# HumanCompatibleAI/overcooked_ai

Measured on NVIDIA H100. Metric: env-steps/sec (joint transitions), higher is better.
Workload: dtype int32

## Files before the change

include/ovc_b200.h:

```cpp
#ifndef OVC_B200_H
#define OVC_B200_H

#include <stddef.h>
#include <stdint.h>

#ifdef __cplusplus
extern "C" {
#endif

#define OVC_ABI_VERSION 5

#define OVC_A_NORTH 0
#define OVC_A_SOUTH 1
#define OVC_A_EAST 2
#define OVC_A_WEST 3
#define OVC_A_STAY 4
#define OVC_A_INTERACT 5
#define OVC_NUM_ACTIONS 6

#define OVC_T_FLOOR 0
#define OVC_T_COUNTER 1
#define OVC_T_ONION 2
#define OVC_T_TOMATO 3
#define OVC_T_DISH 4
// ... 229 lines not shown
} ovc_episode_stats_t;
int ovc_record_transition_stats(const int32_t *sparse, const int32_t *shaped, const int32_t *done, const float *factor, int64_t n_envs,
                                float *rewards, uint8_t *dones, int64_t *ret_sparse, float *ret_mixed, const ovc_episode_stats_t *stats,
                                void *stream);

int ovc_policy_tail(const void *x, int64_t n_rows, int k0, float in_slope, const void *w_first, const float *b_first,
                    const void *w_hidden, const float *b_hidden, int n_hidden, const void *w_heads, const float *b_heads,
                    float slope, int n_actions, uint64_t seed, uint64_t *counter, int32_t *actions, float *values,
                    float *scores, void *stream);
int ovc_policy_tail_logp(const void *x, int64_t n_rows, int k0, float in_slope, const void *w_first, const float *b_first,
                         const void *w_hidden, const float *b_hidden, int n_hidden, const void *w_heads, const float *b_heads,
                         float slope, int n_actions, uint64_t seed, uint64_t *counter, int32_t *actions, float *values,
                         float *scores, float *logp, void *stream);
int ovc_policy_hidden(const void *x, int64_t n_rows, int k0, float in_slope, const void *w_first, const float *b_first,
                      const void *w_hidden, const float *b_hidden, int n_hidden, float slope, void *hidden, void *stream);
int ovc_policy_tail_view(const void *x, int64_t n_rows, int k0, float in_slope, const void *w_first, const float *b_first,
                         const void *w_hidden, const float *b_hidden, int n_hidden, const void *w_heads, const float *b_heads,
                         float slope, int n_actions, uint64_t seed, uint64_t *counter, const int32_t *swap, int seat, int32_t *actions,
                         float *values, float *scores, float *logp, void *stream);

int ovc_lstm_head(const void *x, const void *h_in, const float *c_in, const int32_t *reset, int64_t n_rows, const void *w,
                  const float *b, const void *w_heads, const float *b_heads, int n_actions, uint64_t seed, uint64_t *counter,
                  void *h_out, float *c_out, void *snap_h, float *snap_c, int32_t *actions, float *values, float *logp,
                  float *scores, void *stream);
int ovc_lstm_head_view(const void *x, const void *h_in, const float *c_in, const int32_t *reset, int64_t n_rows, const void *w,
                       const float *b, const void *w_heads, const float *b_heads, int n_actions, uint64_t seed, uint64_t *counter,
                       const int32_t *swap, int seat, void *h_out, float *c_out, void *snap_h, float *snap_c, int32_t *actions,
                       float *values, float *logp, float *scores, void *stream);
int ovc_record_transition_view(const int32_t *sparse, const int32_t *shaped, const int32_t *done, const float *factor, int64_t n_envs,
                               const int32_t *swap, int seat, float *rewards, uint8_t *dones, int64_t *ret_sparse, float *ret_mixed,
                               const ovc_episode_stats_t *stats, void *stream);
int ovc_gae_view(const float *rewards, const float *values, const uint8_t *dones, const float *last_values, int64_t n_steps,
                 int64_t n_envs, float gamma, float lambda, float *advantages, float *value_targets, void *stream);

int ovc_wide_layers(const void *a0, int64_t m, int k0, const void *w1, const float *b1, int n1, const void *w2, const float *b2,
                    int n2, float slope, void *z2, void *stream);

int ovc_partner_policy(const void *layouts, int n_layouts, const void *lut, const int32_t *state, const int32_t *partner_seat,
                       int64_t n_envs, int state_words, int n_features, int width, const void *w_first, const float *b_first,
                       const void *w_hidden, const float *b_hidden, int n_hidden, const void *w_heads, const float *b_heads, int n_actions,
                       uint64_t seed, uint64_t *counter, int32_t *actions, float *scores, void *stream);
int ovc_assign_partners(const int32_t *done, const float *bc_factor, int64_t n_envs, uint64_t seed, uint64_t *counter, int32_t *partner_seat,
                        void *stream);

int ovc_featurize(const void *layouts, int n_layouts, const void *lut, const int32_t *state,
                  const int32_t *view_swap, float *out, int64_t n_envs, int state_words, int num_pots,
                  void *stream);

int ovc_potential(const void *layouts, int n_layouts, const void *pot_tables, const void *cost_lut,
                  const double *gpow, int n_pow, const int32_t *state, double *out, int64_t n_envs,
                  int state_words, void *stream);
size_t ovc_potential_table_size(void);

#ifdef __cplusplus
}
#endif
#endif
```

overcooked_ai_b200/_native.py:

```python
import ctypes
import os

_HERE = os.path.dirname(os.path.abspath(__file__))
LIB_PATH = os.environ.get("OVC_B200_LIB") or os.path.join(_HERE, "csrc", "libovc_b200.so")

ABI_VERSION = 5
F_AUTO_RESET = 1
F_PDL = 2
F_ACT_U8 = 4
F_OUT_NARROW = 8
F_OUT_PACKED = 16
F_OUT_CODES = 32
F_ACT_PACKED = 64
F_OUT_STREAM = 128
F_STREAM_CAP_SHIFT = 16
STREAM_CAP_MAX = 0xFFFF
F_IO_SHIFT = 8
IO_DEFAULT, IO_TMA_TENSOR, IO_TMA_BULK, IO_DIRECT = 0, 1, 2, 3
DT_F32, DT_U8, DT_I32, DT_BF16 = 0, 1, 2, 3



class RandomStart(ctypes.Structure):
    _fields_ = [("seed", ctypes.c_uint64), ("obj_threshold", ctypes.c_uint32), ("random_start_pos", ctypes.c_int32),
# ... 24 lines not shown
    pass


def lib():
    global _lib
    if _lib is not None:
        return _lib
    if not os.path.exists(LIB_PATH):
        raise NativeLibraryError(
            "%s not found: the CUDA extension is not built (python -m overcooked_ai_b200.build). "
            "This engine has no CPU fallback." % LIB_PATH
        )
    L = ctypes.CDLL(LIB_PATH)
    vp, i32, i64 = ctypes.c_void_p, ctypes.c_int, ctypes.c_int64
    L.ovc_abi_version.restype = i32
    L.ovc_layout_table_size.restype = ctypes.c_size_t
    L.ovc_feat_lut_entry_size.restype = ctypes.c_size_t
    L.ovc_last_error.restype = ctypes.c_char_p
    L.ovc_step.argtypes = [vp, i32, vp, vp, vp, vp, vp, vp, vp, i64, i32, i32, i32, vp, vp]
    L.ovc_rollout.argtypes = [vp, i32, vp, vp, vp, vp, vp, vp, vp, i64, i32, i32, i32, i32, vp, vp]
    L.ovc_reset.argtypes = [vp, i32, vp, vp, vp, vp, i64, i32, vp, vp]
    L.ovc_encode_lossless.argtypes = [vp, i32, vp, vp, vp, i32, i64, i32, i32, i32, i32, vp]
    L.ovc_encode_linear.argtypes = [vp, i32, vp, vp, vp, vp, vp, i64, i32, i32, i32, i32, i32, ctypes.c_float, vp]
    L.ovc_sample_actions.argtypes = [vp, i32, i32, i64, ctypes.c_uint64, vp, vp, vp]
    L.ovc_accumulate_returns.argtypes = [vp, vp, ctypes.c_float, i64, vp, vp, vp]
    L.ovc_policy_tail.argtypes = [vp, i64, i32, ctypes.c_float, vp, vp, vp, vp, i32, vp, vp, ctypes.c_float, i32, ctypes.c_uint64, vp, vp, vp, vp, vp]
    L.ovc_policy_tail_logp.argtypes = L.ovc_policy_tail.argtypes[:-1] + [vp, vp]
    L.ovc_policy_hidden.argtypes = [vp, i64, i32, ctypes.c_float, vp, vp, vp, vp, i32, ctypes.c_float, vp, vp]
    L.ovc_lstm_head.argtypes = [vp, vp, vp, vp, i64, vp, vp, vp, vp, i32, ctypes.c_uint64, vp, vp, vp, vp, vp, vp, vp, vp, vp, vp]
    L.ovc_sample_actions_logp.argtypes = [vp, i32, i32, i64, ctypes.c_uint64, vp, vp, vp, vp]
    L.ovc_encode_linear_view.argtypes = [vp, i32, vp, vp, i32, vp, vp, vp, i64, i32, i32, i32, i32, i32, ctypes.c_float, vp]
    L.ovc_sample_actions_view.argtypes = [vp, i32, i32, i64, ctypes.c_uint64, vp, vp, i32, vp, vp, vp]
    L.ovc_policy_tail_view.argtypes = L.ovc_policy_tail.argtypes[:15] + [vp, i32, vp, vp, vp, vp, vp]
    L.ovc_lstm_head_view.argtypes = L.ovc_lstm_head.argtypes[:12] + [vp, i32] + L.ovc_lstm_head.argtypes[12:]
    L.ovc_record_transition.argtypes = [vp, vp, vp, vp, i64, vp, vp, vp, vp, vp]
    L.ovc_record_transition_stats.argtypes = [vp, vp, vp, vp, i64, vp, vp, vp, vp, ctypes.POINTER(EpisodeStatsDesc), vp]
    L.ovc_gae.argtypes = [vp, vp, vp, vp, i64, i64, ctypes.c_float, ctypes.c_float, vp, vp, vp]
    L.ovc_record_transition_view.argtypes = [vp, vp, vp, vp, i64, vp, i32, vp, vp, vp, vp, ctypes.POINTER(EpisodeStatsDesc), vp]
    L.ovc_gae_view.argtypes = L.ovc_gae.argtypes
    L.ovc_wide_layers.argtypes = [vp, i64, i32, vp, vp, i32, vp, vp, i32, ctypes.c_float, vp, vp]
    L.ovc_featurize.argtypes = [vp, i32, vp, vp, vp, vp, i64, i32, i32, vp]
    L.ovc_partner_policy.argtypes = [vp, i32, vp, vp, vp, i64, i32, i32, i32, vp, vp, vp, vp, i32, vp, vp, i32, ctypes.c_uint64, vp, vp, vp, vp]
    L.ovc_assign_partners.argtypes = [vp, vp, i64, ctypes.c_uint64, vp, vp, vp]
    L.ovc_potential.argtypes = [vp, i32, vp, vp, vp, i32, vp, vp, i64, i32, vp]
    L.ovc_potential_table_size.restype = ctypes.c_size_t
    L.ovc_expand_codes_host.argtypes = [vp, i64, i64, vp, vp, i32, vp, vp, vp, vp, i32]
    L.ovc_expand_stream_host.argtypes = [vp, vp, i64, i64, i64, i64, vp, vp, i32, vp, vp, vp, vp, i32, ctypes.POINTER(i64)]
    L.ovc_pipeline_create.argtypes = [ctypes.POINTER(PipelineDesc), ctypes.POINTER(vp)]
    L.ovc_pipeline_run.argtypes = [vp, vp, vp, vp, vp, vp, i32, vp, i32, ctypes.POINTER(i64)]
    L.ovc_pipeline_wait.argtypes = [vp, i64]
    L.ovc_pipeline_join.argtypes = [vp, vp]
    L.ovc_pipeline_destroy.argtypes = [vp]
    L.ovc_pipeline_destroy.restype = None
    for f in (L.ovc_step, L.ovc_rollout, L.ovc_reset, L.ovc_encode_lossless, L.ovc_encode_linear, L.ovc_sample_actions, L.ovc_accumulate_returns, L.ovc_policy_tail, L.ovc_wide_layers, L.ovc_featurize, L.ovc_potential,
              L.ovc_policy_tail_logp, L.ovc_policy_hidden, L.ovc_lstm_head,
              L.ovc_encode_linear_view, L.ovc_sample_actions_view, L.ovc_policy_tail_view, L.ovc_lstm_head_view, L.ovc_sample_actions_logp, L.ovc_record_transition, L.ovc_record_transition_stats, L.ovc_gae, L.ovc_record_transition_view, L.ovc_gae_view, L.ovc_partner_policy, L.ovc_assign_partners, L.ovc_expand_codes_host, L.ovc_expand_stream_host, L.ovc_pipeline_create, L.ovc_pipeline_run, L.ovc_pipeline_wait, L.ovc_pipeline_join):
        f.restype = i32
    if L.ovc_abi_version() != ABI_VERSION:
        raise NativeLibraryError("ABI version mismatch: library %d, binding %d" % (L.ovc_abi_version(), ABI_VERSION))
    _lib = L
    return L


EXPORTED_SYMBOLS = (
    "ovc_abi_version", "ovc_layout_table_size", "ovc_feat_lut_entry_size", "ovc_last_error",
    "ovc_step", "ovc_rollout", "ovc_reset", "ovc_encode_lossless", "ovc_encode_linear", "ovc_sample_actions", "ovc_accumulate_returns", "ovc_policy_tail", "ovc_wide_layers", "ovc_featurize", "ovc_potential",
    "ovc_potential_table_size", "ovc_expand_codes_host", "ovc_expand_stream_host",
    "ovc_policy_tail_logp", "ovc_sample_actions_logp", "ovc_record_transition", "ovc_record_transition_stats", "ovc_gae",
    "ovc_partner_policy", "ovc_assign_partners", "ovc_policy_hidden", "ovc_lstm_head",
    "ovc_encode_linear_view", "ovc_sample_actions_view", "ovc_policy_tail_view", "ovc_lstm_head_view",
    "ovc_record_transition_view", "ovc_gae_view",
    "ovc_pipeline_create", "ovc_pipeline_run", "ovc_pipeline_wait", "ovc_pipeline_join", "ovc_pipeline_destroy",
)


def check(rc):
    if rc != 0:
        raise RuntimeError("ovc native call failed (%d): %s" % (rc, lib().ovc_last_error().decode()))
```

overcooked_ai_b200/batched.py:

```python
import ctypes

import numpy as np
import torch

from overcooked_ai_b200 import _native
from overcooked_ai_b200 import layout as L

_TORCH_DT = {torch.float32: _native.DT_F32, torch.uint8: _native.DT_U8, torch.int32: _native.DT_I32,
             torch.bfloat16: _native.DT_BF16}


def _as_layouts(layouts, mdp_params):
    if isinstance(layouts, (str, L.CompiledLayout)) or hasattr(layouts, "compiled"):
        layouts = [layouts]
    out = []
    for l in layouts:
        if isinstance(l, str):
            l = L.compile_layout(l, **(mdp_params or {}))
        elif hasattr(l, "compiled"):
            l = l.compiled
        out.append(l)
    return out


class BatchedOvercookedEnv(object):
    def __init__(self, layouts, n_envs, horizon=400, device="cuda", auto_reset=False, state_words=None,
                 io=_native.IO_DEFAULT, env_layout=None, mdp_params=None, pdl=True,
                 random_start_pos=False, rnd_obj_prob_thresh=0.0, seed=0, random_layout=False):
        self._lib = _native.lib()
        if not torch.cuda.is_available():
            raise RuntimeError("BatchedOvercookedEnv needs a CUDA device: this engine has no CPU fallback")
        self.device = torch.device(device)
        if self.device.type != "cuda":
            raise ValueError("device must be a CUDA device")
        if self.device.index is None:
            self.device = torch.device("cuda", torch.cuda.current_device())
        self.layouts = _as_layouts(layouts, mdp_params)
        self.n_layouts = len(self.layouts)
        self._longest_cook = max(int(l.cook_time.max()) for l in self.layouts)
        self.n_envs = int(n_envs)
        self.horizon = int(horizon) if horizon < 2**31 else 0
        self.auto_reset = bool(auto_reset)
        self.io = int(io)
        self.pdl = bool(pdl)
        tab, starts, S = L.build_tables(self.layouts, state_words)
        assert tab.shape[1] == self._lib.ovc_layout_table_size(), "layout table size mismatch with the native library"
        self.state_words = S
        self._tab_host, self._starts_host = tab, starts
        with torch.cuda.device(self.device):
            self.tables = torch.from_numpy(tab).to(self.device)
            self.start_records = torch.from_numpy(starts).to(self.device)
            if env_layout is None:
# ... 65 lines not shown
        return (self.n_envs + 31) // 32

    def alloc_stream_out(self, T, cap, n_chunks=1, pin=False, dense_backup=False):
        G = self.n_groups()
        mk = (lambda sh, dt: torch.zeros(sh, dtype=dt, pin_memory=True)) if pin else (lambda sh, dt: torch.zeros(sh, dtype=dt, device=self.device))
        return (mk((T, G), torch.int32), mk((n_chunks, G, cap), torch.int16), mk((T, self.n_envs), torch.int16) if dense_backup else None)

    def rollout_stream(self, actions, cap, out=None, dense_backup=False):
        act_flag = self._action_flag(actions)
        T = actions.shape[0]
        assert 1 <= cap <= _native.STREAM_CAP_MAX
        if out is None:
            out = self.alloc_stream_out(T, cap, dense_backup=dense_backup)
        masks, values, dense = out
        assert masks.dtype == torch.int32 and tuple(masks.shape) == (T, self.n_groups()) and masks.is_cuda and masks.is_contiguous()
        assert values.dtype == torch.int16 and values.numel() == self.n_groups() * cap and values.is_cuda and values.is_contiguous()
        flags = self._flags() | act_flag | _native.F_OUT_STREAM | (int(cap) << _native.F_STREAM_CAP_SHIFT)
        if flags >= 2**31:
            flags -= 2**32
        _native.check(self._lib.ovc_rollout(
            self.tables.data_ptr(), self.n_layouts, self.start_records.data_ptr(), self.state.data_ptr(),
            actions.data_ptr(), values.data_ptr(), 0, 0 if dense is None else dense.data_ptr(), masks.data_ptr(),
            self.n_envs, T, self.state_words, self.horizon, flags, self._rs_ptr(), self._stream()))
        return out

    def expand_stream(self, masks, values, chunk=None, sparse=True, shaped=True, done=True, events=False, n_threads=0, out=None):
        assert masks.dtype == torch.int32 and not masks.is_cuda and masks.is_contiguous() and masks.dim() == 2
        assert values.dtype == torch.int16 and not values.is_cuda and values.is_contiguous() and values.dim() == 3
        T, G = masks.shape
        assert G == self.n_groups() and values.shape[1] == G
        chunk = T if chunk is None else int(chunk)
        assert values.shape[0] == -(-T // chunk)
        out, tbl, lay, ptrs = self._dense_host_out(T, out, sparse, shaped, done, events)
        over = ctypes.c_int64(0)
        _native.check(self._lib.ovc_expand_stream_host(
            masks.data_ptr(), values.data_ptr(), T, chunk, values.shape[2], self.n_envs, lay, tbl.ctypes.data, self.n_layouts, *ptrs,
            int(n_threads), ctypes.byref(over)))
        return out, int(over.value)

    def _dense_host_out(self, T, out, sparse, shaped, done, events):
        tbl = np.ascontiguousarray(self.code_reward_table(), dtype=np.int32)
        lay = self.env_layout_host.ctypes.data
        if self.random_layout:
            assert (tbl == tbl[:1]).all(), "random_layout with different reward tables: the codes alone do not name the layout"
            lay = 0
        if out is None:
            N = self.n_envs
            want = (("sparse", sparse, (T, N), torch.int16), ("shaped", shaped, (T, N, 2), torch.int8),
                    ("done", done, (T, N), torch.uint8), ("events", events, (T, N, 2), torch.int32))
            out = {k: torch.empty(shape, dtype=dt) for k, on, shape, dt in want if on}
        ptrs = [out[k].data_ptr() if k in out else 0 for k in ("sparse", "shaped", "done", "events")]
        return out, tbl, lay, ptrs

    def alloc_rollout_out(self, T, narrow=False, pin=False, packed=False, codes=False):
        N = self.n_envs
        mk = (lambda sh, dt: torch.empty(sh, dtype=dt, pin_memory=True)) if pin else (lambda sh, dt: torch.empty(sh, dtype=dt, device=self.device))
        if codes:
            return (None, None, None, mk((T, N), torch.int16))
        if packed:
            return (mk((T, N), torch.int16), mk((T, N, 2), torch.int8), None, mk((T, N), torch.int16))
        dts = (torch.int16, torch.int8, torch.uint8, torch.int32) if narrow else (torch.int32,) * 4
        shapes = ((T, N), (T, N, 2), (T, N), (T, N, 2))
        return tuple(mk(sh, dt) for sh, dt in zip(shapes, dts))

    def _action_flag(self, actions):
        assert actions.dtype in (torch.int32, torch.uint8) and actions.is_cuda and actions.is_contiguous() and actions.dim() in (2, 3)
        assert actions.shape[1] == self.n_envs
        if actions.dim() == 2:
            assert actions.dtype == torch.uint8, "one-byte joint actions are uint8 [T, N]"
            return _native.F_ACT_PACKED
        assert actions.shape[2] == 2
        return _native.F_ACT_U8 if actions.dtype == torch.uint8 else 0

    def rollout(self, actions, out=None):
        flags = self._flags() | self._action_flag(actions)
        T = actions.shape[0]
        if out is None:
            out = self.alloc_rollout_out(T)
        sparse, shaped, done, events = out
        if sparse is None:
            assert shaped is None and done is None and events.dtype == torch.int16 and events.dim() == 2
            assert tuple(events.shape) == (T, self.n_envs) and events.is_cuda and events.is_contiguous()
            flags |= _native.F_OUT_CODES
            _native.check(self._lib.ovc_rollout(
                self.tables.data_ptr(), self.n_layouts, self.start_records.data_ptr(), self.state.data_ptr(),
                actions.data_ptr(), 0, 0, 0, events.data_ptr(), self.n_envs, T, self.state_words, self.horizon, flags,
                self._rs_ptr(), self._stream()))
            return out
        if done is None:
            assert sparse.dtype == torch.int16 and shaped.dtype == torch.int8 and events.dtype == torch.int16 and events.dim() == 2
            assert self.narrow_ok(), "rewards of these layouts do not fit the narrow formats"
            flags |= _native.F_OUT_PACKED
        elif sparse.dtype == torch.int16:
            assert shaped.dtype == torch.int8 and done.dtype == torch.uint8 and events.dtype == torch.int32
            assert self.narrow_ok(), "rewards of these layouts do not fit the narrow formats"
            flags |= _native.F_OUT_NARROW
        else:
            assert sparse.dtype == shaped.dtype == done.dtype == events.dtype == torch.int32
        _native.check(self._lib.ovc_rollout(
            self.tables.data_ptr(), self.n_layouts, self.start_records.data_ptr(), self.state.data_ptr(),
            actions.data_ptr(), sparse.data_ptr(), shaped.data_ptr(), 0 if done is None else done.data_ptr(), events.data_ptr(),
            self.n_envs, T, self.state_words, self.horizon, flags, self._rs_ptr(), self._stream()))
        return out

    def code_reward_table(self):
        from overcooked_ai_b200 import wire

        return wire.code_reward_table(self.layouts)

    def expand_codes(self, evcode, sparse=True, shaped=True, done=True, events=False, n_threads=0, out=None):
        assert evcode.dtype == torch.int16 and not evcode.is_cuda and evcode.is_contiguous() and evcode.dim() == 2
        T, N = evcode.shape
        assert N == self.n_envs
        out, tbl, lay, ptrs = self._dense_host_out(T, out, sparse, shaped, done, events)
        _native.check(self._lib.ovc_expand_codes_host(evcode.data_ptr(), T, N, lay, tbl.ctypes.data, self.n_layouts, *ptrs, int(n_threads)))
        return out
# ... 261 lines not shown
        rec = (events >> L.EV_RECIPE_SHIFT) & 15
        ids = self.env_layout if layout_ids is None else layout_ids
        lid = ids.long().view(*([1] * (events.dim() - 2)), -1, 1).expand_as(rec)
        return val[lid, rec.long()] * ((events >> 15) & 1)

    def get_states(self, indices=None):
        recs = self.state.cpu().numpy()
        idx = range(self.n_envs) if indices is None else indices
        return [L.unpack_state(self.layouts[int(recs[i][3]) & 0xFF], recs[i]) for i in idx]

    def set_states(self, states, indices=None):
        idx = list(range(self.n_envs)) if indices is None else list(indices)
        lids = self._layout_ids_host()
        recs = np.stack([L.pack_state(self.layouts[lids[i]], s, int(lids[i]), self.state_words) for i, s in zip(idx, states)])
        self.state[torch.as_tensor(idx, device=self.device)] = torch.from_numpy(recs).to(self.device)


class PassTicket(object):

    def __init__(self, pipe, ticket):
        self._pipe, self.ticket = pipe, ticket

    def synchronize(self):
        _native.check(self._pipe._lib.ovc_pipeline_wait(self._pipe._handle, self.ticket))


class HostRolloutPipeline(object):

    def __init__(self, env, n_steps, chunk=50, narrow=False, packed=False, codes=False, host_buffers=1, stream=False,
                 stream_fill=0.25, packed_actions=True):
        codes = codes or stream
        narrow = narrow or packed or codes
        self.env, self.T, self.chunk, self.narrow, self.packed = env, int(n_steps), int(chunk), bool(narrow), bool(packed)
        self.codes, self.stream = bool(codes), bool(stream)
        self.packed_actions = bool(packed_actions) and self.codes
        if narrow:
            assert env.narrow_ok(), "rewards of these layouts do not fit the narrow formats"
        N, dev = env.n_envs, env.device
        self._lib = env._lib
        self.act_dtype = torch.uint8 if narrow else torch.int32
        self.act_shape = (N,) if self.packed_actions else (N, 2)
        self.n_chunks = -(-self.T // self.chunk)
        self.stream_cap = max(1, min(_native.STREAM_CAP_MAX, int(round(self.chunk * 32 * float(stream_fill))))) if stream else 0
        with torch.cuda.device(dev):
            self.d_act = [torch.empty((self.chunk,) + self.act_shape, dtype=self.act_dtype, device=dev) for _ in range(2)]
            if stream:
                G = env.n_groups()
                self.d_out = [(torch.empty((G, self.stream_cap), dtype=torch.int16, device=dev), None, None,
                               torch.empty((self.chunk, G), dtype=torch.int32, device=dev)) for _ in range(2)]
                self.d_codes_full = [torch.empty((self.T, N), dtype=torch.int16, device=dev) for _ in range(2)]
                self.h_outs = [(torch.zeros((self.n_chunks, G, self.stream_cap), dtype=torch.int16, pin_memory=True), None, None,
                                torch.zeros((self.T, G), dtype=torch.int32, pin_memory=True)) for _ in range(max(1, int(host_buffers)))]
            else:
                self.d_out = [env.alloc_rollout_out(self.chunk, narrow=narrow, packed=packed, codes=codes) for _ in range(2)]
                self.h_outs = [env.alloc_rollout_out(self.T, narrow=narrow, pin=True, packed=packed, codes=codes)
                               for _ in range(max(1, int(host_buffers)))]
        self.h_out = self.h_outs[0]
        self._runs = 0
        self.h2d_bytes_per_step = N * (1 if self.packed_actions else 2) * self.d_act[0].element_size()
        if stream:
            self.d2h_bytes_per_step = (self.h_out[3].numel() * 4 + self.h_out[0].numel() * 2) / float(self.T)
        else:
            self.d2h_bytes_per_step = sum(N * (2 if o.dim() == 3 else 1) * o.element_size() for o in self.h_out if o is not None)
        flags = env._flags() | (_native.F_ACT_PACKED if self.packed_actions else _native.F_ACT_U8 if narrow else 0)
        flags |= (_native.F_OUT_STREAM if stream else _native.F_OUT_CODES if codes else _native.F_OUT_PACKED if packed
                  else _native.F_OUT_NARROW if narrow else 0)
        d = _native.PipelineDesc()
        d.layouts, d.n_layouts, d.state_words = env.tables.data_ptr(), env.n_layouts, env.state_words
        d.start_records, d.state, d.n_envs = env.start_records.data_ptr(), env.state.data_ptr(), N
        d.horizon, d.flags, d.chunk = env.horizon, flags, self.chunk
        d.has_random_start = int(env._rs is not None)
        if env._rs is not None:
            d.random_start = env._rs
        ptr = lambda t: 0 if t is None else t.data_ptr()
        for b in range(2):
            d.d_actions[b] = self.d_act[b].data_ptr()
            d.d_sparse[b], d.d_shaped[b], d.d_done[b], d.d_events[b] = (ptr(t) for t in self.d_out[b])
            d.d_codes_full[b] = self.d_codes_full[b].data_ptr() if stream else 0
        d.stream_cap = self.stream_cap
        h = ctypes.c_void_p()
        with torch.cuda.device(dev):
            _native.check(self._lib.ovc_pipeline_create(ctypes.byref(d), ctypes.byref(h)))
        self._handle = h

    def run(self, actions_host, wait=True):
        assert actions_host.dtype == self.act_dtype and actions_host.is_pinned() and actions_host.is_contiguous()
        assert tuple(actions_host.shape) == (self.T,) + self.act_shape
        h_out = self.h_outs[self._runs % len(self.h_outs)]
        self._last_set = self._runs & 1
        self._runs += 1
        ptr = lambda t: 0 if t is None else t.data_ptr()
        ticket = ctypes.c_int64(-1)
        _native.check(self._lib.ovc_pipeline_run(
            self._handle, actions_host.data_ptr(), ptr(h_out[0]), ptr(h_out[1]), ptr(h_out[2]), ptr(h_out[3]), self.T,
            self.env._stream(), int(bool(wait)), ctypes.byref(ticket)))
        self._last_actions = actions_host
        if wait:
            return h_out
        return h_out, PassTicket(self, ticket.value)

    def expand(self, h_out, codes_set=None, out=None, n_threads=0, **which):
        assert self.stream
        dense, over = self.env.expand_stream(h_out[3], h_out[0], chunk=self.chunk, out=out, n_threads=n_threads, **which)
        self.last_overflow = over
        if over:
            cs = self._last_set if codes_set is None else codes_set
            words = self.d_codes_full[cs].cpu()
# ... 88 lines not shown
```

overcooked_ai_b200/csrc/ovc_b200.cu:

```cuda
#include <cuda.h>
#include <cuda_runtime.h>
#include <stdint.h>
#include <stdio.h>
#include <stdlib.h>
#include <string.h>

#include "../../include/ovc_b200.h"
#include "ovc_step.cuh"

namespace ovc {

static thread_local char g_err[512] = "";

static int fail(int code, const char *msg) {
    snprintf(g_err, sizeof g_err, "%s", msg);
    return code;
}
static int fail(int code, const char *msg, long long value) {
    snprintf(g_err, sizeof g_err, "%s (got %lld)", msg, value);
    return code;
}
static int cuda_fail(cudaError_t e, const char *what) {
    snprintf(g_err, sizeof g_err, "%s: %s", what, cudaGetErrorString(e));
    return OVC_E_CUDA;
// ... 318 lines not shown
    encode_tiled_fn enc = get_encode_fn();
    if (!enc) return fail(OVC_E_CUDA, "cuTensorMapEncodeTiled entry point not available");
    cuuint64_t dims[2] = {(cuuint64_t)C::ROW_WORDS, (cuuint64_t)(n_envs * C::ROWS_PER_ENV)};
    cuuint64_t strides[1] = {(cuuint64_t)C::ROW_WORDS * 4};
    cuuint32_t box[2] = {(cuuint32_t)C::ROW_WORDS, (cuuint32_t)box_rows};
    cuuint32_t estr[2] = {1, 1};
    CUresult r = enc(m, CU_TENSOR_MAP_DATA_TYPE_INT32, 2, state, dims, strides, box, estr, CU_TENSOR_MAP_INTERLEAVE_NONE,
                     S == 16 ? CU_TENSOR_MAP_SWIZZLE_64B : CU_TENSOR_MAP_SWIZZLE_128B, CU_TENSOR_MAP_L2_PROMOTION_NONE,
                     CU_TENSOR_MAP_FLOAT_OOB_FILL_NONE);
    if (r != CUDA_SUCCESS) return fail(OVC_E_CUDA, "cuTensorMapEncodeTiled failed", (long long)r);
    return OVC_OK;
}

struct OutFmt {
    int act, sparse, shaped, done, events;
    bool stream;
    bool missing(const void *act_p, const void *sparse_p, const void *shaped_p, const void *done_p, const void *events_p) const {
        return !act_p || !events_p || (sparse && !sparse_p) || (shaped && !shaped_p) || (done && !stream && !done_p);
    }
    bool wide() const { return act == 8 && sparse == 4; }
};

static OutFmt formats_of(int flags) {
    OutFmt f;
    f.act = (flags & OVC_F_ACT_PACKED) ? 1 : (flags & OVC_F_ACT_U8) ? 2 : 8;
    f.stream = flags & OVC_F_OUT_STREAM;
    if (f.stream) f.sparse = 2, f.shaped = 0, f.done = 2, f.events = 4;
    else if (flags & OVC_F_OUT_CODES) f.sparse = 0, f.shaped = 0, f.done = 0, f.events = 2;
    else if (flags & OVC_F_OUT_PACKED) f.sparse = 2, f.shaped = 2, f.done = 0, f.events = 2;
    else if (flags & OVC_F_OUT_NARROW) f.sparse = 2, f.shaped = 2, f.done = 1, f.events = 8;
    else f.sparse = 4, f.shaped = 8, f.done = 4, f.events = 8;
    return f;
}

template <int S, int IO>
static cudaError_t launch_one(const CUtensorMap &tmap, const StepArgs &a, unsigned grid, size_t smem, cudaStream_t st) {
    using C = Cfg<S>;
    cudaLaunchConfig_t cfg;
    memset(&cfg, 0, sizeof cfg);
    cfg.gridDim = dim3(grid), cfg.blockDim = dim3(C::TILE), cfg.dynamicSmemBytes = smem, cfg.stream = st;
    cudaLaunchAttribute attr[1];
    attr[0].id = cudaLaunchAttributeProgrammaticStreamSerialization;
    attr[0].val.programmaticStreamSerializationAllowed = 1;
    cfg.attrs = attr;
    cfg.numAttrs = (a.flags & OVC_F_PDL) ? 1 : 0;
    const bool wide = formats_of(a.flags).wide();
    if (a.has_rs)
        return wide ? cudaLaunchKernelEx(&cfg, step_kernel<S, IO, true, true>, tmap, a)
                    : cudaLaunchKernelEx(&cfg, step_kernel<S, IO, true, false>, tmap, a);
    return wide ? cudaLaunchKernelEx(&cfg, step_kernel<S, IO, false, true>, tmap, a)
                : cudaLaunchKernelEx(&cfg, step_kernel<S, IO, false, false>, tmap, a);
}

template <int S, int TILE>
static int launch_rollout(const StepArgs &a, cudaStream_t st) {
    using C = RollCfg<S, TILE>;
    CUtensorMap tmap;
    memset(&tmap, 0, sizeof tmap);
    int rc = make_tmap<S>(&tmap, a.state, a.n_envs, C::BOX_ROWS);
    if (rc) return rc;
    const size_t smem = C::smem_bytes(a.n_layouts);
    const OutFmt f = formats_of(a.flags);
    const bool wide = f.wide(), stream = f.stream;
    void (*kern)(const CUtensorMap, const StepArgs) =
        a.has_rs ? (wide ? rollout_kernel<S, TILE, true, FMT_WIDE> : stream ? rollout_kernel<S, TILE, true, FMT_STREAM> : rollout_kernel<S, TILE, true, FMT_HOST>)
                 : (wide ? rollout_kernel<S, TILE, false, FMT_WIDE> : stream ? rollout_kernel<S, TILE, false, FMT_STREAM> : rollout_kernel<S, TILE, false, FMT_HOST>);
    if (smem > 48 * 1024) {
        cudaError_t e = cudaFuncSetAttribute(kern, cudaFuncAttributeMaxDynamicSharedMemorySize, (int)smem);
        if (e != cudaSuccess) return cuda_fail(e, "rollout kernel shared-memory attribute");
    }
    const long long grid = (a.n_envs + TILE - 1) / TILE;
    StepArgs ka = a;
    ka.flags &= ~F_K5_NO_PREFETCH;
#if OVC_K5_PREFETCH > 1
    {
        int dev = 0, n_sm = 0, per_sm = 0;
        cudaError_t e = cudaGetDevice(&dev);
        if (e == cudaSuccess) e = cudaDeviceGetAttribute(&n_sm, cudaDevAttrMultiProcessorCount, dev);
        if (e == cudaSuccess) e = cudaOccupancyMaxActiveBlocksPerMultiprocessor(&per_sm, kern, TILE, smem);
        if (e != cudaSuccess) return cuda_fail(e, "rollout kernel occupancy");
        const long long warps = grid * (TILE / 32);
        if (grid <= (long long)per_sm * n_sm && (warps >= 24LL * n_sm || warps < 12LL * n_sm)) ka.flags |= F_K5_NO_PREFETCH;
    }
#endif
    cudaLaunchConfig_t cfg;
    memset(&cfg, 0, sizeof cfg);
    cfg.gridDim = dim3((unsigned)grid), cfg.blockDim = dim3(TILE), cfg.dynamicSmemBytes = smem, cfg.stream = st;
    cudaLaunchAttribute attr[1];
    attr[0].id = cudaLaunchAttributeProgrammaticStreamSerialization;
    attr[0].val.programmaticStreamSerializationAllowed = 1;
    cfg.attrs = attr;
    cfg.numAttrs = 0;
    cudaError_t e = cudaLaunchKernelEx(&cfg, kern, tmap, ka);
    if (e != cudaSuccess) return cuda_fail(e, "rollout kernel launch");
    return OVC_OK;
}

static int rollout_tile(int S, long long n_envs, int n_layouts) {
    static int forced = -1;
    if (forced < 0) {
        const char *e = getenv("OVC_K5_TILE");
        forced = e ? atoi(e) : 0;
    }
    (void)n_envs;
    if (S > 32) return 64;
    if (forced == 32 || forced == 64 || forced == 128) return forced;
    return n_layouts >= 3 ? 128 : 64;
}

static bool use_rollout_kernel(const StepArgs &a, int io) {
    static int off = -1;
    if (off < 0) {
        const char *e = getenv("OVC_K5_LEGACY");
        off = e && atoi(e) ? 1 : 0;
    }
    const bool stream = a.flags & OVC_F_OUT_STREAM;
    return (!off || stream) && (a.n_steps > 1 || stream) && a.n_steps <= ROLLOUT_MAX_STEPS && io == 1 && a.n_layouts <= MAX_SMEM_LAYOUTS;
}

template <int S>
static int launch_rollout_tiled(const StepArgs &a, cudaStream_t st) {
    if constexpr (S > 32) {
        return launch_rollout<S, 64>(a, st);
    } else {
        switch (rollout_tile(S, a.n_envs, a.n_layouts)) {
        case 32: return launch_rollout<S, 32>(a, st);
        case 64: return launch_rollout<S, 64>(a, st);
        default: return launch_rollout<S, 128>(a, st);
        }
    }
}

template <int S>
static int launch_rollout_any(const StepArgs &a0, cudaStream_t st) {
    long long max_steps = 0xFFFFFFFFLL / a0.n_envs - 1;
    {
        static long long cap = -1;
        if (cap < 0) {
            const char *e = getenv("OVC_K5_MAX_LAUNCH_STEPS");
            cap = e ? atoll(e) : 0;
        }
        if (cap > 0 && cap < max_steps && !(a0.flags & OVC_F_OUT_STREAM)) max_steps = cap;
    }
    if (a0.n_steps <= max_steps) return launch_rollout_tiled<S>(a0, st);
    if (max_steps < 1 || (a0.flags & OVC_F_OUT_STREAM)) return fail(OVC_E_UNSUPPORTED, "rollout too large for one launch (n_steps * n_envs must stay below 2^32)");
    const OutFmt f = formats_of(a0.flags);
    for (long long t0 = 0; t0 < a0.n_steps; t0 += max_steps) {
        StepArgs a = a0;
        const long long off = t0 * a0.n_envs;
        a.n_steps = (int)(a0.n_steps - t0 < max_steps ? a0.n_steps - t0 : max_steps);
        a.actions = reinterpret_cast<const int32_t *>(reinterpret_cast<const char *>(a0.actions) + off * f.act);
        if (a0.sparse) a.sparse = reinterpret_cast<int32_t *>(reinterpret_cast<char *>(a0.sparse) + off * f.sparse);
        if (a0.shaped) a.shaped = reinterpret_cast<int32_t *>(reinterpret_cast<char *>(a0.shaped) + off * f.shaped);
        if (a0.done) a.done = reinterpret_cast<int32_t *>(reinterpret_cast<char *>(a0.done) + off * f.done);
        a.events = reinterpret_cast<int32_t *>(reinterpret_cast<char *>(a0.events) + off * f.events);
        const int rc = launch_rollout_tiled<S>(a, st);
        if (rc) return rc;
    }
    return OVC_OK;
}

template <int S>
static int launch_step(const StepArgs &a, int io, cudaStream_t st) {
    using C = Cfg<S>;
    if (use_rollout_kernel(a, io)) return launch_rollout_any<S>(a, st);
    const unsigned grid = (unsigned)((a.n_envs + C::TILE - 1) / C::TILE);
    CUtensorMap tmap;
    memset(&tmap, 0, sizeof tmap);
    const int n_tbl = a.n_layouts <= MAX_SMEM_LAYOUTS ? a.n_layouts : 0;
    const size_t smem = io == 3 ? 0 : C::TILE_BYTES + (size_t)n_tbl * sizeof(ovc_layout_t) + 16;
    cudaError_t e;
    if (io == 1) {
        int rc = make_tmap<S>(&tmap, a.state, a.n_envs);
        if (rc) return rc;
        e = launch_one<S, 1>(tmap, a, grid, smem, st);
    } else if (io == 2) {
        e = launch_one<S, 2>(tmap, a, grid, smem, st);
    } else {
// ... 1 lines not shown
    }
    if (e != cudaSuccess) return cuda_fail(e, "step kernel launch");
    return OVC_OK;
}

static int check_common(const void *layouts, int n_layouts, const void *state, long long n_envs, int S) {
    if (!layouts || !state) return fail(OVC_E_BADARG, "null pointer argument");
    if (n_layouts <= 0 || n_layouts > 256) return fail(OVC_E_BADARG, "n_layouts must be 1..256", (long long)(n_layouts));
    if (n_envs < 0) return fail(OVC_E_BADARG, "negative n_envs");
    if (S != 16 && S != 32 && S != 64 && S != 128)
        return fail(OVC_E_BADARG, "state_words must be 16, 32, 64 or 128", (long long)(S));
    if (((uintptr_t)state & 15) != 0) return fail(OVC_E_BADARG, "state must be 16-byte aligned");
    return OVC_OK;
}

static int step_impl(const void *layouts, int n_layouts, const int32_t *start_records, int32_t *state,
                     const int32_t *actions, int32_t *sparse, int32_t *shaped, int32_t *done, int32_t *events,
                     long long n_envs, int n_steps, int S, int horizon, int flags, const ovc_random_start_t *rs,
                     void *stream) {
    int rc = check_common(layouts, n_layouts, state, n_envs, S);
    if (rc) return rc;
    const OutFmt f = formats_of(flags);
    if (f.stream && (flags & (OVC_F_OUT_CODES | OVC_F_OUT_PACKED | OVC_F_OUT_NARROW)))
        return fail(OVC_E_BADARG, "OVC_F_OUT_STREAM excludes the other output formats");
    if (!start_records || f.missing(actions, sparse, shaped, done, events)) return fail(OVC_E_BADARG, "null pointer argument");
    if (!f.sparse) sparse = nullptr;
    if (!f.shaped) shaped = nullptr;
    if (!f.done) done = nullptr;
    if (f.stream && (((unsigned)flags >> OVC_F_STREAM_CAP_SHIFT) & 0xFFFFu) == 0)
        return fail(OVC_E_BADARG, "OVC_F_OUT_STREAM needs a capacity in flags bits 16-31");
    auto misaligned = [](const void *p, int bytes) { return bytes > 1 && (uintptr_t)p % (uintptr_t)bytes != 0; };
    if (misaligned(actions, f.act) || misaligned(sparse, f.sparse) || misaligned(shaped, f.shaped) || misaligned(done, f.done) ||
        misaligned(events, f.events))
        return fail(OVC_E_BADARG, "actions / sparse / shaped / done / events must be aligned to their element size");
    if (n_steps < 1) return fail(OVC_E_BADARG, "n_steps must be >= 1");
    if (n_envs == 0) return OVC_OK;
    int io = (flags & OVC_F_IO_MASK) >> OVC_F_IO_SHIFT;
    if (io == 0) io = 1;
    if (io < 1 || io > 3) return fail(OVC_E_BADARG, "unknown record I/O strategy", (long long)(io));
    if (io == 1 && (n_envs * (S / (S == 16 ? 16 : 32))) > 0x7FFFFFFFLL) io = 2;
    if (f.stream && (io != 1 || n_layouts > MAX_SMEM_LAYOUTS || n_steps > ROLLOUT_MAX_STEPS))
        return fail(OVC_E_UNSUPPORTED, "OVC_F_OUT_STREAM needs the rollout kernel: default record I/O, at most 8 layouts");
    StepArgs a{(const ovc_layout_t *)layouts, start_records, state, actions, sparse, shaped, done, events,
               n_envs, n_layouts, n_steps, horizon, flags, rs != nullptr, rs ? *rs : ovc_random_start_t{0, 0, 0}};
    cudaStream_t st = (cudaStream_t)stream;
    switch (S) {
    case 16: return launch_step<16>(a, io, st);
    case 32: return launch_step<32>(a, io, st);
    case 64: return launch_step<64>(a, io, st);
    default: return launch_step<128>(a, io, st);
    }
}

}

#include "ovc_obs.cuh"
#include "ovc_encfc.cuh"
#include "ovc_tail.cuh"
#include "ovc_wide.cuh"
#include "ovc_partner.cuh"
#include "ovc_lstm.cuh"
#include "ovc_potential.cuh"
#include "ovc_host.cuh"

extern "C" {

int ovc_abi_version(void) { return OVC_ABI_VERSION; }
size_t ovc_layout_table_size(void) { return sizeof(ovc_layout_t); }
size_t ovc_feat_lut_entry_size(void) { return sizeof(ovc_feat_lut_entry_t); }
const char *ovc_last_error(void) { return ovc::g_err; }

int ovc_step(const void *layouts, int n_layouts, const int32_t *start_records, int32_t *state, const int32_t *actions,
             int32_t *sparse, int32_t *shaped, int32_t *done, int32_t *events, int64_t n_envs, int state_words,
             int horizon, int flags, const ovc_random_start_t *random_start, void *stream) {
    return ovc::step_impl(layouts, n_layouts, start_records, state, actions, sparse, shaped, done, events, n_envs, 1,
                          state_words, horizon, flags, random_start, stream);
}

int ovc_rollout(const void *layouts, int n_layouts, const int32_t *start_records, int32_t *state,
                const int32_t *actions, int32_t *sparse, int32_t *shaped, int32_t *done, int32_t *events,
                int64_t n_envs, int n_steps, int state_words, int horizon, int flags,
                const ovc_random_start_t *random_start, void *stream) {
    return ovc::step_impl(layouts, n_layouts, start_records, state, actions, sparse, shaped, done, events, n_envs,
                          n_steps, state_words, horizon, flags, random_start, stream);
}

int ovc_reset(const void *layouts, int n_layouts, const int32_t *start_records, int32_t *state, const int32_t *env_layout,
              const int32_t *mask, int64_t n_envs, int state_words, const ovc_random_start_t *random_start, void *stream) {
    int rc = ovc::check_common(layouts, n_layouts, state, n_envs, state_words);
    if (rc) return rc;
    if (!start_records) return ovc::fail(OVC_E_BADARG, "null pointer argument");
    if (n_envs == 0) return OVC_OK;
    const int threads = 256;
    if (random_start) {
        ovc::reset_random_kernel<<<(unsigned)((n_envs + threads - 1) / threads), threads, 0, (cudaStream_t)stream>>>(
            (const ovc_layout_t *)layouts, n_layouts, start_records, state, env_layout, mask, n_envs, state_words,
            *random_start);
    } else {
        const long long chunks = (long long)n_envs * (state_words / 4);
        ovc::reset_kernel<<<(unsigned)((chunks + threads - 1) / threads), threads, 0, (cudaStream_t)stream>>>(
            start_records, n_layouts, state, env_layout, mask, n_envs, state_words);
    }
    cudaError_t e = cudaGetLastError();
    if (e != cudaSuccess) return ovc::cuda_fail(e, "reset kernel launch");
    return OVC_OK;
}
// ... 163 lines not shown
                       int64_t n_envs, int state_words, int n_features, int width, const void *w_first, const float *b_first,
                       const void *w_hidden, const float *b_hidden, int n_hidden, const void *w_heads, const float *b_heads, int n_actions,
                       uint64_t seed, uint64_t *counter, int32_t *actions, float *scores, void *stream) {
    int rc = ovc::check_common(layouts, n_layouts, state, n_envs, state_words);
    if (rc) return rc;
    ovc::PartnerArgs a;
    a.f.layouts = (const ovc_layout_t *)layouts, a.f.lut = (const ovc_feat_lut_entry_t *)lut, a.f.state = state, a.f.view_swap = nullptr;
    a.f.out = nullptr, a.f.n_envs = n_envs, a.f.S = state_words, a.f.num_pots = 2, a.f.B = ovc::PP_B, a.f.F = ovc::PP_F, a.f.E = ovc::FEAT_E;
    a.partner_seat = partner_seat, a.w_first = (const __nv_bfloat16 *)w_first, a.b_first = b_first, a.w_hidden = (const __nv_bfloat16 *)w_hidden;
    a.b_hidden = b_hidden, a.w_heads = (const __nv_bfloat16 *)w_heads, a.b_heads = b_heads, a.n_hidden = n_hidden, a.n_actions = n_actions;
    a.seed = seed, a.counter = (unsigned long long *)counter, a.actions = actions, a.scores = scores;
    return ovc::partner_policy_impl(a, n_features, width, (cudaStream_t)stream);
}

int ovc_assign_partners(const int32_t *done, const float *bc_factor, int64_t n_envs, uint64_t seed, uint64_t *counter, int32_t *partner_seat,
                        void *stream) {
    return ovc::assign_partners_impl(done, bc_factor, n_envs, seed, (unsigned long long *)counter, partner_seat, (cudaStream_t)stream);
}

int ovc_featurize(const void *layouts, int n_layouts, const void *lut, const int32_t *state,
                  const int32_t *view_swap, float *out, int64_t n_envs, int state_words, int num_pots, void *stream) {
    int rc = ovc::check_common(layouts, n_layouts, state, n_envs, state_words);
    if (rc) return rc;
    return ovc::featurize_impl((const ovc_layout_t *)layouts, (const ovc_feat_lut_entry_t *)lut, state, view_swap, out,
                               n_envs, state_words, num_pots, (cudaStream_t)stream);
}

int ovc_potential(const void *layouts, int n_layouts, const void *pot_tables, const void *cost_lut, const double *gpow,
                  int n_pow, const int32_t *state, double *out, int64_t n_envs, int state_words, void *stream) {
    int rc = ovc::check_common(layouts, n_layouts, state, n_envs, state_words);
    if (rc) return rc;
    return ovc::potential_impl((const ovc_layout_t *)layouts, (const ovc_potential_t *)pot_tables,
                               (const ovc_cost_lut_entry_t *)cost_lut, gpow, n_pow, state, out, n_envs, state_words,
                               (cudaStream_t)stream);
}
size_t ovc_potential_table_size(void) { return sizeof(ovc_potential_t); }

int ovc_pipeline_create(const ovc_pipeline_desc_t *desc, ovc_pipeline_t **out) { return ovc::pipeline_create(desc, out); }
int ovc_pipeline_run(ovc_pipeline_t *p, const void *h_actions, void *h_sparse, void *h_shaped, void *h_done, void *h_events,
                     int n_steps, void *stream, int join, int64_t *ticket) {
    if (!p) return ovc::fail(OVC_E_BADARG, "null pipeline");
    return ovc::pipeline_run(p, h_actions, h_sparse, h_shaped, h_done, h_events, n_steps, (cudaStream_t)stream, join, ticket);
}
int ovc_pipeline_wait(ovc_pipeline_t *p, int64_t ticket) {
    if (!p) return ovc::fail(OVC_E_BADARG, "null pipeline");
    return ovc::pipeline_wait(p, ticket);
}
int ovc_pipeline_join(ovc_pipeline_t *p, void *stream) {
    if (!p) return ovc::fail(OVC_E_BADARG, "null pipeline");
    return ovc::pipeline_join(p, (cudaStream_t)stream);
}
void ovc_pipeline_destroy(ovc_pipeline_t *p) { ovc::pipeline_destroy(p); }

int ovc_expand_stream_host(const uint32_t *masks, const uint16_t *values, int64_t n_steps, int64_t chunk, int64_t cap,
                           int64_t n_envs, const int32_t *env_layout, const int32_t *reward_tbl, int n_layouts, int16_t *sparse,
                           int8_t *shaped, uint8_t *done, int32_t *events, int n_threads, int64_t *overflow) {
    return ovc::expand_stream_host(masks, values, n_steps, chunk, cap, n_envs, env_layout, reward_tbl, n_layouts, sparse, shaped,
                                   done, events, n_threads, overflow);
}

int ovc_expand_codes_host(const uint16_t *codes, int64_t n_steps, int64_t n_envs, const int32_t *env_layout,
                          const int32_t *reward_tbl, int n_layouts, int16_t *sparse, int8_t *shaped, uint8_t *done,
                          int32_t *events, int n_threads) {
    return ovc::expand_codes_host(codes, n_steps, n_envs, env_layout, reward_tbl, n_layouts, sparse, shaped, done, events,
                                  n_threads);
}

}
```

Baseline: 76.38 billion.

## Allocate rollout outputs in compressible memory and pick smaller tile for one-wave grids

Adds a CUDA VMM-based allocator that requests generic-compression device memory, exposed to PyTorch through a pluggable MemPool, and routes device rollout output buffers through it by default when the device supports it. The goal is to cut DRAM write bandwidth for the highly compressible int outputs. It also computes occupancy for a 32-thread tile on S=16 with few layouts and switches to that tile when the grid fits in one wave, aiming for better SM spread. The risks are that H100 may not grant compression, that the allocator adds setup cost, and that the smaller tile changes per-CTA efficiency.

```diff
diff --git a/include/ovc_b200.h b/include/ovc_b200.h
--- a/include/ovc_b200.h
+++ b/include/ovc_b200.h
@@ -305,6 +305,10 @@
                   int state_words, void *stream);
 size_t ovc_potential_table_size(void);
 
+int ovc_comp_supported(int device);
+void *ovc_comp_alloc(ptrdiff_t size, int device, void *stream);
+void ovc_comp_free(void *ptr, size_t size, int device, void *stream);
+
 #ifdef __cplusplus
 }
 #endif
diff --git a/overcooked_ai_b200/_native.py b/overcooked_ai_b200/_native.py
--- a/overcooked_ai_b200/_native.py
+++ b/overcooked_ai_b200/_native.py
@@ -100,6 +100,8 @@
     L.ovc_pipeline_join.argtypes = [vp, vp]
     L.ovc_pipeline_destroy.argtypes = [vp]
     L.ovc_pipeline_destroy.restype = None
+    L.ovc_comp_supported.argtypes = [i32]
+    L.ovc_comp_supported.restype = i32
     for f in (L.ovc_step, L.ovc_rollout, L.ovc_reset, L.ovc_encode_lossless, L.ovc_encode_linear, L.ovc_sample_actions, L.ovc_accumulate_returns, L.ovc_policy_tail, L.ovc_wide_layers, L.ovc_featurize, L.ovc_potential,
               L.ovc_policy_tail_logp, L.ovc_policy_hidden, L.ovc_lstm_head,
               L.ovc_encode_linear_view, L.ovc_sample_actions_view, L.ovc_policy_tail_view, L.ovc_lstm_head_view, L.ovc_sample_actions_logp, L.ovc_record_transition, L.ovc_record_transition_stats, L.ovc_gae, L.ovc_record_transition_view, L.ovc_gae_view, L.ovc_partner_policy, L.ovc_assign_partners, L.ovc_expand_codes_host, L.ovc_expand_stream_host, L.ovc_pipeline_create, L.ovc_pipeline_run, L.ovc_pipeline_wait, L.ovc_pipeline_join):
@@ -119,9 +121,35 @@
     "ovc_encode_linear_view", "ovc_sample_actions_view", "ovc_policy_tail_view", "ovc_lstm_head_view",
     "ovc_record_transition_view", "ovc_gae_view",
     "ovc_pipeline_create", "ovc_pipeline_run", "ovc_pipeline_wait", "ovc_pipeline_join", "ovc_pipeline_destroy",
+    "ovc_comp_supported", "ovc_comp_alloc", "ovc_comp_free",
 )
 
 
 def check(rc):
     if rc != 0:
         raise RuntimeError("ovc native call failed (%d): %s" % (rc, lib().ovc_last_error().decode()))
+
+
+_comp_pools = {}
+
+
+def compression_allowed():
+    return os.environ.get("OVC_COMPRESSIBLE", "1") != "0"
+
+
+def compressible_pool(device):
+    if not compression_allowed():
+        return None
+    if device not in _comp_pools:
+        rc = lib().ovc_comp_supported(device)
+        if rc < 0:
+            check(rc)
+        pool = None
+        if rc:
+            import torch
+
+            with torch.cuda.device(device):
+                alloc = torch.cuda.memory.CUDAPluggableAllocator(LIB_PATH, "ovc_comp_alloc", "ovc_comp_free")
+                pool = torch.cuda.MemPool(alloc.allocator())
+        _comp_pools[device] = pool
+    return _comp_pools[device]
diff --git a/overcooked_ai_b200/batched.py b/overcooked_ai_b200/batched.py
--- a/overcooked_ai_b200/batched.py
+++ b/overcooked_ai_b200/batched.py
@@ -1,3 +1,4 @@
+import contextlib
 import ctypes
 
 import numpy as np
@@ -169,16 +170,26 @@
         ptrs = [out[k].data_ptr() if k in out else 0 for k in ("sparse", "shaped", "done", "events")]
         return out, tbl, lay, ptrs
 
-    def alloc_rollout_out(self, T, narrow=False, pin=False, packed=False, codes=False):
+    def outputs_compressible(self):
+        return _native.compressible_pool(self.device.index) is not None
+
+    def alloc_rollout_out(self, T, narrow=False, pin=False, packed=False, codes=False, compressible=None):
         N = self.n_envs
+        pool = None
+        if not pin and compressible is not False:
+            pool = _native.compressible_pool(self.device.index)
+            if pool is None and compressible:
+                raise RuntimeError("compressible outputs requested, but %s does not grant compressible memory "
+                                   "(or OVC_COMPRESSIBLE=0)" % self.device)
         mk = (lambda sh, dt: torch.empty(sh, dtype=dt, pin_memory=True)) if pin else (lambda sh, dt: torch.empty(sh, dtype=dt, device=self.device))
-        if codes:
-            return (None, None, None, mk((T, N), torch.int16))
-        if packed:
-            return (mk((T, N), torch.int16), mk((T, N, 2), torch.int8), None, mk((T, N), torch.int16))
-        dts = (torch.int16, torch.int8, torch.uint8, torch.int32) if narrow else (torch.int32,) * 4
-        shapes = ((T, N), (T, N, 2), (T, N), (T, N, 2))
-        return tuple(mk(sh, dt) for sh, dt in zip(shapes, dts))
+        with torch.cuda.use_mem_pool(pool, self.device) if pool is not None else contextlib.nullcontext():
+            if codes:
+                return (None, None, None, mk((T, N), torch.int16))
+            if packed:
+                return (mk((T, N), torch.int16), mk((T, N, 2), torch.int8), None, mk((T, N), torch.int16))
+            dts = (torch.int16, torch.int8, torch.uint8, torch.int32) if narrow else (torch.int32,) * 4
+            shapes = ((T, N), (T, N, 2), (T, N), (T, N, 2))
+            return tuple(mk(sh, dt) for sh, dt in zip(shapes, dts))
 
     def _action_flag(self, actions):
         assert actions.dtype in (torch.int32, torch.uint8) and actions.is_cuda and actions.is_contiguous() and actions.dim() in (2, 3)
@@ -546,7 +557,8 @@
                 self.h_outs = [(torch.zeros((self.n_chunks, G, self.stream_cap), dtype=torch.int16, pin_memory=True), None, None,
                                 torch.zeros((self.T, G), dtype=torch.int32, pin_memory=True)) for _ in range(max(1, int(host_buffers)))]
             else:
-                self.d_out = [env.alloc_rollout_out(self.chunk, narrow=narrow, packed=packed, codes=codes) for _ in range(2)]
+                self.d_out = [env.alloc_rollout_out(self.chunk, narrow=narrow, packed=packed, codes=codes, compressible=False)
+                              for _ in range(2)]
                 self.h_outs = [env.alloc_rollout_out(self.T, narrow=narrow, pin=True, packed=packed, codes=codes)
                                for _ in range(max(1, int(host_buffers)))]
         self.h_out = self.h_outs[0]
diff --git a/overcooked_ai_b200/csrc/ovc_b200.cu b/overcooked_ai_b200/csrc/ovc_b200.cu
--- a/overcooked_ai_b200/csrc/ovc_b200.cu
+++ b/overcooked_ai_b200/csrc/ovc_b200.cu
@@ -394,6 +394,25 @@
                 : cudaLaunchKernelEx(&cfg, step_kernel<S, IO, false, false>, tmap, a);
 }
 
+typedef void (*rollout_fn)(const CUtensorMap, const StepArgs);
+
+template <int S, int TILE>
+static rollout_fn rollout_kernel_for(const StepArgs &a) {
+    const OutFmt f = formats_of(a.flags);
+    const bool wide = f.wide(), stream = f.stream;
+    return a.has_rs ? (wide ? rollout_kernel<S, TILE, true, FMT_WIDE> : stream ? rollout_kernel<S, TILE, true, FMT_STREAM> : rollout_kernel<S, TILE, true, FMT_HOST>)
+                    : (wide ? rollout_kernel<S, TILE, false, FMT_WIDE> : stream ? rollout_kernel<S, TILE, false, FMT_STREAM> : rollout_kernel<S, TILE, false, FMT_HOST>);
+}
+
+static cudaError_t resident_ctas(rollout_fn kern, int threads, size_t smem, long long *ctas, int *n_sm) {
+    int dev = 0, per_sm = 0;
+    cudaError_t e = cudaGetDevice(&dev);
+    if (e == cudaSuccess) e = cudaDeviceGetAttribute(n_sm, cudaDevAttrMultiProcessorCount, dev);
+    if (e == cudaSuccess) e = cudaOccupancyMaxActiveBlocksPerMultiprocessor(&per_sm, kern, threads, smem);
+    *ctas = (long long)per_sm * *n_sm;
+    return e;
+}
+
 template <int S, int TILE>
 static int launch_rollout(const StepArgs &a, cudaStream_t st) {
     using C = RollCfg<S, TILE>;
@@ -402,11 +421,7 @@
     int rc = make_tmap<S>(&tmap, a.state, a.n_envs, C::BOX_ROWS);
     if (rc) return rc;
     const size_t smem = C::smem_bytes(a.n_layouts);
-    const OutFmt f = formats_of(a.flags);
-    const bool wide = f.wide(), stream = f.stream;
-    void (*kern)(const CUtensorMap, const StepArgs) =
-        a.has_rs ? (wide ? rollout_kernel<S, TILE, true, FMT_WIDE> : stream ? rollout_kernel<S, TILE, true, FMT_STREAM> : rollout_kernel<S, TILE, true, FMT_HOST>)
-                 : (wide ? rollout_kernel<S, TILE, false, FMT_WIDE> : stream ? rollout_kernel<S, TILE, false, FMT_STREAM> : rollout_kernel<S, TILE, false, FMT_HOST>);
+    const rollout_fn kern = rollout_kernel_for<S, TILE>(a);
     if (smem > 48 * 1024) {
         cudaError_t e = cudaFuncSetAttribute(kern, cudaFuncAttributeMaxDynamicSharedMemorySize, (int)smem);
         if (e != cudaSuccess) return cuda_fail(e, "rollout kernel shared-memory attribute");
@@ -416,13 +431,12 @@
     ka.flags &= ~F_K5_NO_PREFETCH;
 #if OVC_K5_PREFETCH > 1
     {
-        int dev = 0, n_sm = 0, per_sm = 0;
-        cudaError_t e = cudaGetDevice(&dev);
-        if (e == cudaSuccess) e = cudaDeviceGetAttribute(&n_sm, cudaDevAttrMultiProcessorCount, dev);
-        if (e == cudaSuccess) e = cudaOccupancyMaxActiveBlocksPerMultiprocessor(&per_sm, kern, TILE, smem);
+        long long resident = 0;
+        int n_sm = 0;
+        cudaError_t e = resident_ctas(kern, TILE, smem, &resident, &n_sm);
         if (e != cudaSuccess) return cuda_fail(e, "rollout kernel occupancy");
         const long long warps = grid * (TILE / 32);
-        if (grid <= (long long)per_sm * n_sm && (warps >= 24LL * n_sm || warps < 12LL * n_sm)) ka.flags |= F_K5_NO_PREFETCH;
+        if (grid <= resident && (warps >= 24LL * n_sm || warps < 12LL * n_sm)) ka.flags |= F_K5_NO_PREFETCH;
     }
 #endif
     cudaLaunchConfig_t cfg;
@@ -438,16 +452,16 @@
     return OVC_OK;
 }
 
-static int rollout_tile(int S, long long n_envs, int n_layouts) {
+static int rollout_tile(int S, int n_layouts, bool one_wave_at_32) {
     static int forced = -1;
     if (forced < 0) {
         const char *e = getenv("OVC_K5_TILE");
         forced = e ? atoi(e) : 0;
     }
-    (void)n_envs;
     if (S > 32) return 64;
     if (forced == 32 || forced == 64 || forced == 128) return forced;
-    return n_layouts >= 3 ? 128 : 64;
+    if (n_layouts >= 3) return 128;
+    return S == 16 && one_wave_at_32 ? 32 : 64;
 }
 
 static bool use_rollout_kernel(const StepArgs &a, int io) {
@@ -465,7 +479,15 @@
     if constexpr (S > 32) {
         return launch_rollout<S, 64>(a, st);
     } else {
-        switch (rollout_tile(S, a.n_envs, a.n_layouts)) {
+        bool one_wave_at_32 = false;
+        if (S == 16 && a.n_layouts < 3) {
+            long long resident = 0;
+            int n_sm = 0;
+            cudaError_t e = resident_ctas(rollout_kernel_for<S, 32>(a), 32, RollCfg<S, 32>::smem_bytes(a.n_layouts), &resident, &n_sm);
+            if (e != cudaSuccess) return cuda_fail(e, "rollout kernel occupancy");
+            one_wave_at_32 = (a.n_envs + 31) / 32 <= resident;
+        }
+        switch (rollout_tile(S, a.n_layouts, one_wave_at_32)) {
         case 32: return launch_rollout<S, 32>(a, st);
         case 64: return launch_rollout<S, 64>(a, st);
         default: return launch_rollout<S, 128>(a, st);
@@ -573,6 +595,151 @@
     }
 }
 
+struct CompDriver {
+    decltype(&cuDeviceGet) device_get = nullptr;
+    decltype(&cuDeviceGetAttribute) device_attribute = nullptr;
+    decltype(&cuMemGetAllocationGranularity) granularity = nullptr;
+    decltype(&cuMemAddressReserve) reserve = nullptr;
+    decltype(&cuMemAddressFree) address_free = nullptr;
+    decltype(&cuMemCreate) create = nullptr;
+    decltype(&cuMemRelease) release = nullptr;
+    decltype(&cuMemMap) map = nullptr;
+    decltype(&cuMemUnmap) unmap = nullptr;
+    decltype(&cuMemSetAccess) set_access = nullptr;
+    decltype(&cuMemGetAllocationPropertiesFromHandle) properties = nullptr;
+    bool ok = false;
+};
+
+template <class F>
+static bool driver_entry(const char *name, F &fn) {
+    void *p = nullptr;
+    cudaDriverEntryPointQueryResult q;
+    if (cudaGetDriverEntryPoint(name, &p, cudaEnableDefault, &q) != cudaSuccess || q != cudaDriverEntryPointSuccess) return false;
+    fn = (F)p;
+    return true;
+}
+
+static const CompDriver &comp_driver() {
+    static const CompDriver d = [] {
+        CompDriver c;
+        c.ok = driver_entry("cuDeviceGet", c.device_get) && driver_entry("cuDeviceGetAttribute", c.device_attribute) &&
+               driver_entry("cuMemGetAllocationGranularity", c.granularity) && driver_entry("cuMemAddressReserve", c.reserve) &&
+               driver_entry("cuMemAddressFree", c.address_free) && driver_entry("cuMemCreate", c.create) &&
+               driver_entry("cuMemRelease", c.release) && driver_entry("cuMemMap", c.map) && driver_entry("cuMemUnmap", c.unmap) &&
+               driver_entry("cuMemSetAccess", c.set_access) &&
+               driver_entry("cuMemGetAllocationPropertiesFromHandle", c.properties);
+        return c;
+    }();
+    return d;
+}
+
+static int drv_fail(CUresult r, const char *what) {
+    snprintf(g_err, sizeof g_err, "%s failed (CUresult %d)", what, (int)r);
+    return OVC_E_CUDA;
+}
+
+static CUmemAllocationProp comp_prop(CUdevice dev) {
+    CUmemAllocationProp p;
+    memset(&p, 0, sizeof p);
+    p.type = CU_MEM_ALLOCATION_TYPE_PINNED;
+    p.location.type = CU_MEM_LOCATION_TYPE_DEVICE;
+    p.location.id = (int)dev;
+    p.allocFlags.compressionType = CU_MEM_ALLOCATION_COMP_GENERIC;
+    return p;
+}
+
+static int comp_device(int device, CUdevice *dev, size_t *gran) {
+    const CompDriver &d = comp_driver();
+    if (!d.ok) return fail(OVC_E_CUDA, "the driver's virtual memory management entry points are not available");
+    CUresult r = d.device_get(dev, device);
+    if (r != CUDA_SUCCESS) return drv_fail(r, "cuDeviceGet");
+    CUmemAllocationProp p = comp_prop(*dev);
+    r = d.granularity(gran, &p, CU_MEM_ALLOC_GRANULARITY_MINIMUM);
+    return r == CUDA_SUCCESS ? OVC_OK : drv_fail(r, "cuMemGetAllocationGranularity");
+}
+
+static int comp_probe(int device) {
+    int prev = 0;
+    cudaError_t e = cudaGetDevice(&prev);
+    if (e == cudaSuccess) e = cudaSetDevice(device);
+    if (e == cudaSuccess) e = cudaFree(nullptr);
+    if (e != cudaSuccess) return cuda_fail(e, "compressible memory probe");
+    const CompDriver &d = comp_driver();
+    CUdevice dev;
+    size_t gran = 0;
+    int rc = comp_device(device, &dev, &gran);
+    int attr = 0;
+    if (rc == OVC_OK) {
+        CUresult r = d.device_attribute(&attr, CU_DEVICE_ATTRIBUTE_GENERIC_COMPRESSION_SUPPORTED, dev);
+        if (r != CUDA_SUCCESS) rc = drv_fail(r, "cuDeviceGetAttribute");
+    }
+    if (rc == OVC_OK && attr) {
+        CUmemAllocationProp p = comp_prop(dev);
+        CUmemGenericAllocationHandle h;
+        CUresult r = d.create(&h, gran, &p, 0);
+        if (r == CUDA_SUCCESS) {
+            CUmemAllocationProp got;
+            memset(&got, 0, sizeof got);
+            r = d.properties(&got, h);
+            attr = r == CUDA_SUCCESS && got.allocFlags.compressionType == CU_MEM_ALLOCATION_COMP_GENERIC;
+            d.release(h);
+        } else {
+            attr = 0;
+        }
+    }
+    cudaSetDevice(prev);
+    return rc == OVC_OK ? attr : rc;
+}
+
+static void *comp_alloc(size_t size, int device) {
+    const CompDriver &d = comp_driver();
+    CUdevice dev;
+    size_t gran = 0;
+    if (comp_device(device, &dev, &gran) != OVC_OK) return nullptr;
+    size_t padded = (size + gran - 1) / gran * gran;
+    CUdeviceptr ptr = 0;
+    CUresult r = d.reserve(&ptr, padded, gran, 0, 0);
+    if (r != CUDA_SUCCESS) return drv_fail(r, "cuMemAddressReserve"), nullptr;
+    CUmemAllocationProp p = comp_prop(dev);
+    CUmemGenericAllocationHandle h;
+    r = d.create(&h, padded, &p, 0);
+    if (r != CUDA_SUCCESS) {
+        d.address_free(ptr, padded);
+        return drv_fail(r, "cuMemCreate"), nullptr;
+    }
+    r = d.map(ptr, padded, 0, h, 0);
+    d.release(h);
+    if (r != CUDA_SUCCESS) {
+        d.address_free(ptr, padded);
+        return drv_fail(r, "cuMemMap"), nullptr;
+    }
+    CUmemAccessDesc acc;
+    acc.location = p.location;
+    acc.flags = CU_MEM_ACCESS_FLAGS_PROT_READWRITE;
+    r = d.set_access(ptr, padded, &acc, 1);
+    if (r != CUDA_SUCCESS) {
+        d.unmap(ptr, padded);
+        d.address_free(ptr, padded);
+        return drv_fail(r, "cuMemSetAccess"), nullptr;
+    }
+    return (void *)ptr;
+}
+
+static void comp_free(void *ptr, size_t size, int device) {
+    const CompDriver &d = comp_driver();
+    CUdevice dev;
+    size_t gran = 0;
+    if (!ptr || comp_device(device, &dev, &gran) != OVC_OK) return;
+    size_t padded = (size + gran - 1) / gran * gran;
+    int prev = 0;
+    if (cudaGetDevice(&prev) == cudaSuccess && cudaSetDevice(device) == cudaSuccess) {
+        cudaDeviceSynchronize();
+        cudaSetDevice(prev);
+    }
+    d.unmap((CUdeviceptr)ptr, padded);
+    d.address_free((CUdeviceptr)ptr, padded);
+}
+
 }
 
 #include "ovc_obs.cuh"
@@ -842,6 +1009,19 @@
 }
 void ovc_pipeline_destroy(ovc_pipeline_t *p) { ovc::pipeline_destroy(p); }
 
+int ovc_comp_supported(int device) {
+    static int known[64];
+    if (device < 0 || device >= 64) return ovc::fail(OVC_E_BADARG, "device ordinal out of range", device);
+    if (known[device] == 0) {
+        int rc = ovc::comp_probe(device);
+        if (rc < 0) return rc;
+        known[device] = rc + 1;
+    }
+    return known[device] - 1;
+}
+void *ovc_comp_alloc(ptrdiff_t size, int device, void *) { return size > 0 ? ovc::comp_alloc((size_t)size, device) : nullptr; }
+void ovc_comp_free(void *ptr, size_t size, int device, void *) { ovc::comp_free(ptr, size, device); }
+
 int ovc_expand_stream_host(const uint32_t *masks, const uint16_t *values, int64_t n_steps, int64_t chunk, int64_t cap,
                            int64_t n_envs, const int32_t *env_layout, const int32_t *reward_tbl, int n_layouts, int16_t *sparse,
                            int8_t *shaped, uint8_t *done, int32_t *events, int n_threads, int64_t *overflow) {
```

Measured after the change: 80.66 billion (median of 6 runs). +5.6%, better.
